# mpsops/mps-bitsandbytes

Measured on AMD Instinct MI355X. Metric: effective bf16 TFLOPS, NF4 dequant+matmul 4096x4096 @ M=4096 (dequantise-once + dense GEMM, two launches), higher is better.
Workload: dtype bf16

## Files before the change

mps_bitsandbytes_amd/csrc/common.h:

```cpp
#pragma once

#include <hip/hip_runtime.h>
#include <stdint.h>

#include "../../include/mbnb_hip.h"
#include "elem_types.h"

namespace mbnb {

template <int DT> struct ElemT;
template <> struct ElemT<MBNB_F16> { using type = f16_t; };
template <> struct ElemT<MBNB_BF16> { using type = bf16_t; };
template <> struct ElemT<MBNB_F32> { using type = float; };

template <typename T> __device__ __forceinline__ float to_f32(T v) { return (float)v; }
template <typename T> __device__ __forceinline__ T from_f32(float v) { return (T)v; }
template <> __device__ __forceinline__ f16_t from_f32<f16_t>(float v) {
    asm("" : "+v"(v));
    return (f16_t)v;
}

typedef uint32_t u32x4 __attribute__((ext_vector_type(4)));
typedef uint32_t u32x2 __attribute__((ext_vector_type(2)));
typedef float f32x4 __attribute__((ext_vector_type(4)));
// ... 15 lines not shown
template <> __device__ __forceinline__ uint32_t pack2<bf16_t>(float lo, float hi) {
    bf16x2 v = {(bf16_t)lo, (bf16_t)hi};
    return __builtin_bit_cast(uint32_t, v);
}

template <typename T> __device__ __forceinline__ float unpack_lo(uint32_t w);
template <typename T> __device__ __forceinline__ float unpack_hi(uint32_t w);
template <> __device__ __forceinline__ float unpack_lo<f16_t>(uint32_t w) {
    return (float)__builtin_bit_cast(f16x2, w)[0];
}
template <> __device__ __forceinline__ float unpack_hi<f16_t>(uint32_t w) {
    return (float)__builtin_bit_cast(f16x2, w)[1];
}
template <> __device__ __forceinline__ float unpack_lo<bf16_t>(uint32_t w) {
    return __builtin_bit_cast(float, w << 16);
}
template <> __device__ __forceinline__ float unpack_hi<bf16_t>(uint32_t w) {
    return __builtin_bit_cast(float, w & 0xFFFF0000u);
}

__device__ __forceinline__ float nf4_code(int i) {
    constexpr float t[16] = {-1.0f, -0.6961928009986877f, -0.5250730514526367f, -0.39491748809814453f,
                             -0.28444138169288635f, -0.18477343022823334f, -0.09105003625154495f, 0.0f,
                             0.07958029955625534f, 0.16093020141124725f, 0.24611230194568634f,
                             0.33791524171829224f, 0.44070982933044434f, 0.5626170039176941f,
                             0.7229568362236023f, 1.0f};
    return t[i];
}
__device__ __forceinline__ float fp4_code(int i) {
    constexpr float t[16] = {0.0f, 0.0625f, 0.125f, 0.25f, 0.375f, 0.5f, 0.75f, 1.0f,
                             -0.0f, -0.0625f, -0.125f, -0.25f, -0.375f, -0.5f, -0.75f, -1.0f};
    return t[i];
}
template <int QT> __device__ __forceinline__ float code_value(int i) {
    return QT == MBNB_NF4 ? nf4_code(i) : fp4_code(i);
}

template <int QT> __device__ __forceinline__ void fill_code_lut(float *lut, int tid) {
    if (tid < 16) {
        float v = 0.0f;
#pragma unroll
        for (int i = 0; i < 16; i++)
            if (tid == i) v = code_value<QT>(i);
        lut[tid] = v;
    }
}

constexpr int W8_INT8 = 0, W8_FP8 = 1;

__device__ __forceinline__ float fp8_e4m3_to_float(uint32_t b) {
    const uint32_t t = b << 24;
    const uint32_t u = (t & 0x80000000u) | ((t >> 4) & 0x07F00000u);
    float f = __builtin_bit_cast(float, u) * 0x1p120f;
    if ((t & 0x7F000000u) == 0x7F000000u) f = __builtin_bit_cast(float, 0x7FC00000u);
    return f;
}

__device__ __forceinline__ int fp8_exponent(float a) {
    const uint32_t u = __builtin_bit_cast(uint32_t, a);
    const uint32_t ef = (u >> 23) & 0xFFu;
    if (ef == 0) return -127;
    int e = (int)ef - 127;
    const int k = e + 1;
    const uint32_t n = k >= 9 ? 5u : k >= 5 ? 2u : k >= 3 ? 1u : k >= -1 ? 0u : k >= -3 ? 1u : k >= -7 ? 2u : k >= -15 ? 5u : 11u;
    if ((0x7FFFFFu - (u & 0x7FFFFFu)) < n) e += 1;
    return e;
}

__device__ __forceinline__ uint32_t float_to_fp8_e4m3(float v) {
    if (v != v) return 0x7Fu;
    const uint32_t sign = v < 0.0f ? 0x80u : 0u;
    const uint32_t ab = __builtin_bit_cast(uint32_t, fminf(fabsf(v), 448.0f));
    if (ab == 0u) return sign;
    const int k = (int)(ab >> 23) - 126;
    const uint32_t m = ab & 0x7FFFFFu;
    const int t = 2 * k - 1, at = t < 0 ? -t : t;
    const uint32_t n = at >= 9 ? 2u : (at >= 5 ? 1u : 0u);
    const bool bump = (0x7FFFFFu - m) < n;
    const int biased = k + 6 + (bump ? 1 : 0);
    if (biased >= 15) return sign | 0x77u;
    if (biased <= 0) return sign;
    uint32_t mb = (m + 0x80000u) >> 20;
    mb = bump ? 0u : (mb > 7u ? 7u : mb);
    return sign | ((uint32_t)biased << 3) | mb;
}

struct OutlierEpilogue {
    const void *x;
    int64_t ldx;
    const int64_t *oidx;
    int64_t n_out;
    const void *ow;
    const void *bias;
};

template <int WF> __device__ __forceinline__ float w8_row_scale(float s) { return WF == W8_INT8 ? s / 127.0f : s; }
template <int WF> __device__ __forceinline__ float w8_decode(uint32_t byte) {
    if constexpr (WF == W8_INT8) return (float)(int)(int8_t)byte;
    else return fp8_e4m3_to_float(byte);
}
template <int WF> __device__ __forceinline__ float w8_decode_sel(uint32_t word, int sel) {
    if constexpr (WF == W8_INT8) {
        return (float)(int)(int8_t)(word >> (8 * sel));
    } else {
        switch (sel) {
            case 0: return __builtin_amdgcn_cvt_f32_fp8((int)word, 0);
            case 1: return __builtin_amdgcn_cvt_f32_fp8((int)word, 1);
            case 2: return __builtin_amdgcn_cvt_f32_fp8((int)word, 2);
            default: return __builtin_amdgcn_cvt_f32_fp8((int)word, 3);
        }
    }
}

struct AbsmaxView {
    const float *f32;
    const int8_t *i8;
    const float *am2;
    int bs2;
};

template <bool NESTED> __device__ __forceinline__ float load_absmax(const AbsmaxView &a, int64_t i) {
    if constexpr (NESTED) {
        float s = a.am2[i / a.bs2] / 127.0f;
        return (float)a.i8[i] * s;
    } else {
        return a.f32[i];
    }
}

__device__ __forceinline__ float rscale127(float absmax) {
    float r = 1.0f / absmax;
    return r * 127.0f;
}

__device__ __forceinline__ int8_t quant_i8(float x, float scale) {
    float q = rintf(x * scale);
    q = fminf(fmaxf(q, -127.0f), 127.0f);
    return (int8_t)(int)q;
}

__device__ __forceinline__ float wave_max(float v) {
#pragma unroll
    for (int off = 32; off > 0; off >>= 1) v = fmaxf(v, __shfl_xor(v, off, 64));
    return v;
}
__device__ __forceinline__ float wave_sum(float v) {
#pragma unroll
    for (int off = 32; off > 0; off >>= 1) v += __shfl_xor(v, off, 64);
    return v;
}

constexpr int MBNB_NOT_APPLICABLE = -1000;

__device__ __forceinline__ void store_f32x4_wt(float *dst, f32x4 v) { asm volatile("global_store_dwordx4 %0, %1, off sc1" ::"v"(dst), "v"(v) : "memory"); }
__device__ __forceinline__ void store_out16_nt(u32x4 *dst, u32x4 v) { __builtin_nontemporal_store(v, dst); }
__device__ __forceinline__ void store_out16(u32x4 *dst, u32x4 v) {
    asm volatile("global_store_dwordx4 %0, %1, off sc1" ::"v"(dst), "v"(v) : "memory");
}
void set_error(const char *fmt, ...);
void set_kernel_name(const char *name);
void set_kernel_variant(const char *fmt, ...) __attribute__((format(printf, 1, 2)));
int check_launch(const char *what);
int ensure_dyn_lds(const void *func, int bytes, const char *what);

}
```

mps_bitsandbytes_amd/csrc/gemm_dense.h:

```cpp
#pragma once
#include "gemm256.h"
#include <type_traits>
#include <utility>

namespace mbnb {

template <int... I, class F> __device__ __forceinline__ void gd_static_for_impl(std::integer_sequence<int, I...>, F &&f) {
    (f(std::integral_constant<int, I>{}), ...);
}
template <int N, class F> __device__ __forceinline__ void gd_static_for(F &&f) {
    gd_static_for_impl(std::make_integer_sequence<int, N>{}, static_cast<F &&>(f));
}

constexpr int GD_LDS = 4 * P_IMG;

template <int FM, int FN = 8> struct GdPlan {
    static_assert(FN == 8 || (FM == 8 && FN >= 5 && FN <= 7), "narrow tiles exist for the 256-row tile only");
    static constexpr int NS = 2 * FN * FM, NR = FN + FM, NP = FN + FM;
    static constexpr int RS1 = (FM == 8 && FN >= 7) ? 2 : 1;
    static constexpr int B1 = FM != 8 ? 16 : (FN == 8 ? 36 : FN == 7 ? 32 : FN == 6 ? 16 : 13), D0 = B1;
    static constexpr int DS = FM == 8 ? 4 : 2;
    static constexpr int B2 = FM != 8 ? 42 : (FN == 8 ? 100 : FN == 7 ? 94 : FN == 6 ? 78 : 66), R0 = B2;
    static_assert(R0 >= FN * FM, "the next tile's slice 0 replaces this tile's only after its MFMAs");
    static_assert((NR - 1) * RS1 < B1, "slice 1 is in registers before barrier 1");
// ... 45 lines not shown

    typedef int i32x4_t __attribute__((ext_vector_type(4)));
    i32x4_t rs_a, rs_b;
    {
        const uint64_t pa = reinterpret_cast<uint64_t>(X + m0 * K + k_begin), pb = reinterpret_cast<uint64_t>(Wd + n0 * ldw + k_begin);
        const int64_t rows_a = M - m0 < TM ? M - m0 : TM, rows_b = N - n0 < TN ? N - n0 : TN;
        rs_a = i32x4_t{(int)(uint32_t)pa, (int)(uint32_t)(pa >> 32), (int)(rows_a * K * 2), 0x00020000};
        rs_b = i32x4_t{(int)(uint32_t)pb, (int)(uint32_t)(pb >> 32), (int)(rows_b * ldw * 2), 0x00020000};
    }
    int voff_a[FM], voff_b[FN];
#pragma unroll
    for (int pl = 0; pl < FN; pl++) {
        const int row = 8 * (FN * wave + pl) + (lane >> 3);
        voff_b[pl] = (int)(row * ldw * 2) + 16 * ((lane & 7) ^ ((row >> 1) & 7));
    }
#pragma unroll
    for (int pl = 0; pl < FM; pl++) {
        const int row = 8 * (FM * wave + pl) + (lane >> 3);
        voff_a[pl] = (int)(row * K * 2) + 16 * ((lane & 7) ^ ((row >> 1) & 7));
    }
#pragma unroll
    for (int pl = 0; pl < FN; pl++) voff_b[pl] -= (pl & 3) * 1024;
#pragma unroll
    for (int pl = 0; pl < FM; pl++) voff_a[pl] -= (pl & 3) * 1024;
    const uint32_t smem_base = (uint32_t)(uintptr_t)(__attribute__((address_space(3))) void *)smem;
    struct DmaCtx { i32x4_t ra, rb; uint32_t lwa, lwb; };
    auto dma_ctx = [&]() {
        DmaCtx c;
#pragma unroll
        for (int e = 0; e < 4; e++) {
            c.ra[e] = __builtin_amdgcn_readfirstlane(rs_a[e]);
            c.rb[e] = __builtin_amdgcn_readfirstlane(rs_b[e]);
        }
        c.lwa = (uint32_t)__builtin_amdgcn_readfirstlane((int)(smem_base + (uint32_t)(P_A + wave * FM * 1024)));
        c.lwb = (uint32_t)__builtin_amdgcn_readfirstlane((int)(smem_base + (uint32_t)(P_B + wave * FN * 1024)));
        return c;
    };
    auto issue_piece = [&](auto qq, int stage, int kb, const DmaCtx &c) {
        constexpr int q = decltype(qq)::value, pl = q < FM ? q : q - FM;
        const uint32_t dst = (q < FM ? c.lwa : c.lwb) + (uint32_t)(stage * P_IMG + pl * 1024);
        const int vo = (q < FM) ? voff_a[pl] : voff_b[pl];
        const i32x4_t rs = (q < FM) ? c.ra : c.rb;
        if constexpr ((pl & 3) != 0) {
            asm volatile("buffer_load_dwordx4 %0, %1, %2 offen offset:%3 lds" ::"v"(vo), "s"(rs), "s"(kb), "n"((pl & 3) * 1024) : "memory", "m0");
        } else {
            asm volatile("s_mov_b32 m0, %0\n\ts_nop 0\n\tbuffer_load_dwordx4 %1, %2, %3 offen lds" ::"s"(dst), "v"(vo), "s"(rs), "s"(kb) : "memory", "m0");
        }
    };

    const int r16 = lane & 15, fq = lane >> 4;
    int fw[2], fx[2];
#pragma unroll
    for (int ks = 0; ks < 2; ks++) {
        const int f = r16 * ROW_BYTES + (((4 * ks + fq) ^ (r16 >> 1)) << 4);
        fw[ks] = P_B + wn * 16 * FN * ROW_BYTES + f;
        fx[ks] = P_A + wm * 16 * FM * ROW_BYTES + f;
    }
    Frag wf[2][FN], xf[2][FM];
    auto read_one = [&](int stage, auto kk, auto nn) {
        constexpr int ks = decltype(kk)::value, n = decltype(nn)::value;
        if constexpr (n == 0) wf[ks][0] = *reinterpret_cast<const Frag *>(smem + fw[ks] + stage * P_IMG);
        else if constexpr (n <= FM) xf[ks][n - 1] = *reinterpret_cast<const Frag *>(smem + fx[ks] + stage * P_IMG + (n - 1) * 16 * ROW_BYTES);
        else wf[ks][n - FM] = *reinterpret_cast<const Frag *>(smem + fw[ks] + stage * P_IMG + (n - FM) * 16 * ROW_BYTES);
    };
    f32x4 acc[FN][FM];

    auto kbytes = [&](int t) { return t << 7; };

    {
        const DmaCtx c0 = dma_ctx();
        gd_static_for<Plan::NP>([&](auto q) { issue_piece(q, 0, 0, c0); });
        if (nk > 1) {
            gd_static_for<Plan::NP>([&](auto q) { issue_piece(q, 1, kbytes(1), c0); });
            asm volatile("s_waitcnt vmcnt(%0)" ::"n"(Plan::NP) : "memory");
        } else {
            asm volatile("s_waitcnt vmcnt(0)" ::: "memory");
        }
    }
    __builtin_amdgcn_s_barrier();
    asm volatile("" ::: "memory");
    gd_static_for<Plan::NR>([&](auto n) { read_one(0, std::integral_constant<int, 0>{}, n); });

    auto mfma_acc = [&](f32x4 &c, const Frag &a, const Frag &b) {
        if constexpr (I8) asm volatile("v_mfma_i32_16x16x64_i8 %0, %1, %2, %0" : "+a"(c) : "v"(a), "v"(b));
        else if constexpr (std::is_same_v<T, bf16_t>) asm volatile("v_mfma_f32_16x16x32_bf16 %0, %1, %2, %0" : "+a"(c) : "v"(a), "v"(b));
        else asm volatile("v_mfma_f32_16x16x32_f16 %0, %1, %2, %0" : "+a"(c) : "v"(a), "v"(b));
    };
    auto mfma_zero = [&](f32x4 &c, const Frag &a, const Frag &b) {
        if constexpr (I8) asm volatile("v_mfma_i32_16x16x64_i8 %0, %1, %2, 0" : "=a"(c) : "v"(a), "v"(b));
        else if constexpr (std::is_same_v<T, bf16_t>) asm volatile("v_mfma_f32_16x16x32_bf16 %0, %1, %2, 0" : "=a"(c) : "v"(a), "v"(b));
        else asm volatile("v_mfma_f32_16x16x32_f16 %0, %1, %2, 0" : "=a"(c) : "v"(a), "v"(b));
    };

    auto kstep = [&](auto cc, auto first, auto mode_, auto wo_, int j, const DmaCtx &dc) {
        constexpr int WO = decltype(wo_)::value, MODE = decltype(mode_)::value;
        constexpr bool FIRST = decltype(first)::value;
        const int C = cc, Nn = C ^ 1;
        int kb2 = 0;
        if constexpr (MODE == 0) kb2 = __builtin_amdgcn_readfirstlane(kbytes(j + 2));
        gd_static_for<Plan::NS>([&](auto tt) {
            constexpr int t = decltype(tt)::value, ks = t / (FN * FM), f = (t % (FN * FM)) / FM, g = t % FM;
            if constexpr (t == Plan::B1 && MODE != 2) {
                asm volatile("s_waitcnt lgkmcnt(0)" ::: "memory");
                __builtin_amdgcn_s_barrier();
                asm volatile("" ::: "memory");
            }
            if constexpr (t == Plan::B2 && MODE != 2) {
                asm volatile("s_waitcnt vmcnt(%0)" ::"n"(MODE == 0 ? Plan::NP : 0) : "memory");
                __builtin_amdgcn_s_barrier();
                asm volatile("" ::: "memory");
            }
            if constexpr (FIRST && ks == 0) mfma_zero(acc[f][g], wf[ks][f], xf[ks][g]);
            else mfma_acc(acc[f][g], wf[ks][f], xf[ks][g]);
            if constexpr ((t % Plan::RS1) == 0 && t / Plan::RS1 < Plan::NR)
                read_one(C, std::integral_constant<int, 1>{}, std::integral_constant<int, (t / Plan::RS1) % Plan::NR>{});
            if constexpr (MODE != 2 && t >= Plan::R0 && t < Plan::R0 + Plan::NR)
                read_one(Nn, std::integral_constant<int, 0>{}, std::integral_constant<int, (t - Plan::R0) % Plan::NR>{});
            if constexpr (MODE == 0 && t >= Plan::D0 && t < Plan::D0 + Plan::NP * Plan::DS && ((t - Plan::D0) % Plan::DS) == WO)
                issue_piece(std::integral_constant<int, ((t - Plan::D0) / Plan::DS) % Plan::NP>{}, C, kb2, dc);
            __builtin_amdgcn_sched_barrier(0);
        });
    };
    using Mode0 = std::integral_constant<int, 0>;
    using Mode1 = std::integral_constant<int, 1>;
    using Mode2 = std::integral_constant<int, 2>;
    auto main_loop = [&](auto wo) {
        if (nk < 3) return;
        const DmaCtx dc = dma_ctx();
        kstep(std::integral_constant<int, 0>{}, std::true_type{}, Mode0{}, wo, 0, dc);
        int j = 1;
        for (; j + 3 < nk; j += 2) {
            kstep(std::integral_constant<int, 1>{}, std::false_type{}, Mode0{}, wo, j, dc);
            kstep(std::integral_constant<int, 0>{}, std::false_type{}, Mode0{}, wo, j + 1, dc);
        }
        if (j + 2 < nk) kstep(std::integral_constant<int, 1>{}, std::false_type{}, Mode0{}, wo, j, dc);
    };
    if constexpr (Plan::DS == 4) {
        if (wave == 0) main_loop(std::integral_constant<int, 0>{});
        else if (wave == 1) main_loop(std::integral_constant<int, 1>{});
        else if (wave == 2) main_loop(std::integral_constant<int, 2>{});
        else main_loop(std::integral_constant<int, 3>{});
    } else {
        if ((wave & 1) == 0) main_loop(std::integral_constant<int, 0>{});
        else main_loop(std::integral_constant<int, 1>{});
    }

    constexpr bool TAIL = !SPLITK && !I8 && OUTL == 0 && FN == 8;
    bool tail_ok = false;
    if constexpr (TAIL)
        tail_ok = nk >= 2 && out_dtype == (std::is_same_v<T, f16_t> ? MBNB_F16 : MBNB_BF16) && (N % 8 == 0) &&
                  ((reinterpret_cast<uintptr_t>(out_v) & 15) == 0) && N < ((int64_t)1 << 23);
    u32x2 bias_t[TAIL ? FN : 1];
    if constexpr (TAIL) {
        if (tail_ok && bias != nullptr) {
            const uint16_t *bp = reinterpret_cast<const uint16_t *>(bias);
#pragma unroll
            for (int f = 0; f < FN; f++) {
                const int64_t n = n0 + wn * 16 * FN + 16 * f + 4 * fq;
                if (n + 4 <= N && (reinterpret_cast<uintptr_t>(bp + n) & 7) == 0) bias_t[f] = *reinterpret_cast<const u32x2 *>(bp + n);
                else {
                    uint32_t t[4];
#pragma unroll
                    for (int e = 0; e < 4; e++) t[e] = bp[n + e < N ? n + e : N - 1];
                    bias_t[f] = u32x2{t[0] | (t[1] << 16), t[2] | (t[3] << 16)};
                }
            }
        }
    }
    {
        const DmaCtx none{};
        if (nk == 2) kstep(std::integral_constant<int, 0>{}, std::true_type{}, Mode1{}, std::integral_constant<int, 0>{}, 0, none);
        else if (nk > 2) kstep(nk & 1, std::false_type{}, Mode1{}, std::integral_constant<int, 0>{}, nk - 2, none);
        if (nk == 1) kstep(std::integral_constant<int, 0>{}, std::true_type{}, Mode2{}, std::integral_constant<int, 0>{}, 0, none);
        else if (!tail_ok) kstep((nk - 1) & 1, std::false_type{}, Mode2{}, std::integral_constant<int, 0>{}, nk - 1, none);
    }
    if constexpr (TAIL) {
        auto tail_step = [&](auto wb_t, const int C) {
            constexpr bool WB = decltype(wb_t)::value;
            constexpr int ROWB = 264, GS = 2 * FN;
            int tid2 = threadIdx.x;
            asm volatile("" : "+v"(tid2));
            const int lane_e = tid2 & 63, er16 = lane_e & 15, efq = lane_e >> 4;
            char *stg = smem + (wn ? P_B : P_A) + (C ^ 1) * P_IMG + wm * (2 * 16 * ROWB);
            char *st_w = stg + er16 * ROWB + 8 * efq;
            const char *st_r = stg + efq * ROWB + er16 * 16;
            const int64_t m_w = m0 + wm * 16 * FM;
            int64_t rows = M - m_w;
            rows = rows < 0 ? 0 : (rows > 16 * FM ? 16 * FM : rows);
            const uint64_t po = reinterpret_cast<uint64_t>(static_cast<uint16_t *>(out_v) + m_w * N);
            i32x4_t rs_o;
            rs_o[0] = __builtin_amdgcn_readfirstlane((int)(uint32_t)po);
            rs_o[1] = __builtin_amdgcn_readfirstlane((int)(uint32_t)(po >> 32));
            rs_o[2] = __builtin_amdgcn_readfirstlane((int)(rows * N * 2));
            rs_o[3] = 0x00020000;
            const int rowstep = __builtin_amdgcn_readfirstlane((int)(N * 2));
            const int64_t n = n0 + wn * 16 * FN + er16 * 8;
            const int voff0 = n < N ? (int)((efq * N + n) * 2) : (int)0x80000000;
            u32x4 piece[4];
            auto filler = [&](auto gg, auto ss) {
                constexpr int g = decltype(gg)::value, s = decltype(ss)::value, buf = (g & 1) * 16 * ROWB;
                if constexpr (s < FN) {
                    float bv[4] = {0.0f, 0.0f, 0.0f, 0.0f};
                    if constexpr (WB) {
#pragma unroll
                        for (int e = 0; e < 4; e++) bv[e] = unpack_lo<T>(bias_t[s][e >> 1] >> (16 * (e & 1)));
                    }
                    float v[4];
#pragma unroll
                    for (int e = 0; e < 4; e++) {
                        float sv;
                        asm volatile("v_accvgpr_read_b32 %0, %1" : "=v"(sv) : "a"(acc[s][g][e]));
                        v[e] = sv + bv[e];
                    }
                    const u32x2 pk = u32x2{pack2<T>(v[0], v[1]), pack2<T>(v[2], v[3])};
                    *reinterpret_cast<u32x2 *>(st_w + buf + 32 * s) = pk;
                } else if constexpr (s < FN + 4) {
                    constexpr int p = s - FN;
                    const char *srcp = st_r + buf + p * 4 * ROWB;
                    const u32x2 lo = *reinterpret_cast<const u32x2 *>(srcp), hi = *reinterpret_cast<const u32x2 *>(srcp + 8);
                    piece[p] = u32x4{lo[0], lo[1], hi[0], hi[1]};
                } else if constexpr (s < FN + 8) {
                    constexpr int p = s - FN - 4;
                    const int vo = voff0 + (16 * g + 4 * p) * rowstep;
                    const i32x4_t rs = rs_o;
                    const u32x4 pv = piece[p];
                    asm volatile("buffer_store_dwordx4 %0, %1, %2, 0 offen sc1\n\ts_nop 1" ::"v"(pv), "v"(vo), "s"(rs) : "memory");
                }
            };
            gd_static_for<Plan::NS>([&](auto tt) {
                constexpr int t = decltype(tt)::value, g = t / GS, ks = (t % GS) / FN, f = t % FN;
                if constexpr (std::is_same_v<T, bf16_t>) asm volatile("s_nop 1\n\tv_mfma_f32_16x16x32_bf16 %0, %1, %2, %0" : "+a"(acc[f][g]) : "v"(wf[ks][f]), "v"(xf[ks][g]));
                else asm volatile("s_nop 1\n\tv_mfma_f32_16x16x32_f16 %0, %1, %2, %0" : "+a"(acc[f][g]) : "v"(wf[ks][f]), "v"(xf[ks][g]));
                if constexpr (t < Plan::NR)
                    read_one(C, std::integral_constant<int, 1>{},
                             std::integral_constant<int, (t == 0 ? 1 : t == 1 ? 0 : t <= FN ? t - 1 + FM : t - FN + 1)>{});
                if constexpr (t >= GS) filler(std::integral_constant<int, t / GS - 1>{}, std::integral_constant<int, t % GS>{});
                __builtin_amdgcn_sched_barrier(0);
            });
            gd_static_for<GS>([&](auto ss) {
                filler(std::integral_constant<int, FM - 1>{}, ss);
                __builtin_amdgcn_sched_barrier(0);
            });
        };
        if (tail_ok) {
            if (bias != nullptr) tail_step(std::true_type{}, (nk - 1) & 1);
            else tail_step(std::false_type{}, (nk - 1) & 1);
            return;
        }
    }

    asm volatile("s_waitcnt lgkmcnt(0)" ::: "memory");
    __builtin_amdgcn_s_barrier();
    asm volatile("" ::: "memory");
    int tid2 = threadIdx.x;
    asm volatile("" : "+v"(tid2));
    const int lane_e = tid2 & 63, er16 = lane_e & 15, efq = lane_e >> 4;
    const int64_t n_base = n0 + wn * 16 * FN;
    if constexpr (SPLITK) {
        float *o = partial + (int64_t)slice * M * N;
#pragma unroll
        for (int f = 0; f < FN; f++)
#pragma unroll
            for (int g = 0; g < FM; g++) {
                const int64_t m = m0 + wm * 16 * FM + 16 * g + er16, nn = n_base + 16 * f + 4 * efq;
                float v[4];
#pragma unroll
                for (int e = 0; e < 4; e++) asm volatile("v_accvgpr_read_b32 %0, %1" : "=v"(v[e]) : "a"(acc[f][g][e]));
                if (m < M && nn < N) store4_partial(o + m * N + nn, v, nn, N);
                __builtin_amdgcn_sched_barrier(0);
            }
        return;
    }
    if (out_dtype == MBNB_F32) {
        float *o = static_cast<float *>(out_v);
#pragma unroll
        for (int f = 0; f < FN; f++)
#pragma unroll
            for (int g = 0; g < FM; g++) {
                const int64_t m = m0 + wm * 16 * FM + 16 * g + er16, nn = n_base + 16 * f + 4 * efq;
                float v[4];
#pragma unroll
                for (int e = 0; e < 4; e++) {
                    float sv;
                    asm volatile("v_accvgpr_read_b32 %0, %1" : "=v"(sv) : "a"(acc[f][g][e]));
                    if constexpr (I8) {
                        v[e] = (float)__builtin_bit_cast(int, sv) * (sA[m < M ? m : M - 1] / 127.0f) * (sB[nn + e < N ? nn + e : N - 1] / 127.0f);
                    } else {
                        if (bias != nullptr && nn + e < N) sv += to_f32(bias[nn + e]);
                        v[e] = to_f32(from_f32<T>(sv));
                    }
                }
                if (m < M && nn < N) store4(o + m * N + nn, v, nn, N);
                __builtin_amdgcn_sched_barrier(0);
            }
        return;
    }
    constexpr int ROWB = 264;
    char *wave_lds = smem + wave * 64 * ROWB;
    uint16_t *out = static_cast<uint16_t *>(out_v);
    const bool vec_ok = (N % 8 == 0) && ((reinterpret_cast<uintptr_t>(out_v) & 15) == 0);
    const bool same_out = !I8 && out_dtype == (std::is_same_v<T, f16_t> ? MBNB_F16 : MBNB_BF16);
    const bool with_outl = OUTL != 0 && ep.x != nullptr && ep.n_out > 0;
    const bool ow_vec = OUTL != 0 && (ep.n_out % 8 == 0) && ((reinterpret_cast<uintptr_t>(ep.ow) & 15) == 0);
    using OutlT = std::conditional_t<OUTL == 1, f16_t, bf16_t>;
    auto rne = [&](float x) { return to_f32(from_f32<OutlT>(x)); };
    u32x4 wfr_all[OUTL ? 8 * NCH : 1];
    u32x2 bias_all[(OUTL || !I8) ? FN : 1];
    u32x4 xfr_all[OUTL ? FM * NCH : 1];
    if constexpr (!I8) {
        if (bias != nullptr) {
            const uint16_t *bp = reinterpret_cast<const uint16_t *>(bias);
#pragma unroll
            for (int f = 0; f < FN; f++) {
                const int64_t n = n_base + 16 * f + 4 * efq;
                if (n + 4 <= N && (reinterpret_cast<uintptr_t>(bp + n) & 7) == 0) bias_all[f] = *reinterpret_cast<const u32x2 *>(bp + n);
                else {
                    uint32_t t[4];
#pragma unroll
                    for (int e = 0; e < 4; e++) t[e] = bp[n + e < N ? n + e : N - 1];
                    bias_all[f] = u32x2{t[0] | (t[1] << 16), t[2] | (t[3] << 16)};
                }
            }
        }
    }
    if constexpr (OUTL) {
#pragma unroll
        for (int f = 0; f < 8; f++) {
            bias_all[f] = u32x2{0u, 0u};
#pragma unroll
            for (int c = 0; c < NCH; c++) {
                wfr_all[8 * c + f] = u32x4{0u, 0u, 0u, 0u};
                if (with_outl) {
                    const uint16_t *ow = static_cast<const uint16_t *>(ep.ow);
                    int64_t n = n_base + 16 * f + er16;
                    n = n < N ? n : N - 1;
                    const int64_t j0 = 32 * c + 8 * efq;
                    if (ow_vec && j0 + 8 <= ep.n_out) wfr_all[8 * c + f] = *reinterpret_cast<const u32x4 *>(ow + n * ep.n_out + j0);
                    else if (j0 < ep.n_out) {
                        uint32_t t[8];
#pragma unroll
                        for (int e = 0; e < 8; e++) t[e] = (j0 + e < ep.n_out) ? (uint32_t)ow[n * ep.n_out + j0 + e] : 0u;
                        wfr_all[8 * c + f] = u32x4{t[0] | (t[1] << 16), t[2] | (t[3] << 16), t[4] | (t[5] << 16), t[6] | (t[7] << 16)};
                    }
                }
            }
            if (ep.bias != nullptr) {
                const uint16_t *bp = static_cast<const uint16_t *>(ep.bias);
                const int64_t n = n_base + 16 * f + 4 * efq;
                if (n + 4 <= N && (reinterpret_cast<uintptr_t>(bp + n) & 7) == 0) bias_all[f] = *reinterpret_cast<const u32x2 *>(bp + n);
                else {
                    uint32_t t[4];
#pragma unroll
                    for (int e = 0; e < 4; e++) t[e] = bp[n + e < N ? n + e : N - 1];
                    bias_all[f] = u32x2{t[0] | (t[1] << 16), t[2] | (t[3] << 16)};
                }
            }
        }
#pragma unroll
        for (int g = 0; g < FM; g++) {
#pragma unroll
            for (int c = 0; c < NCH; c++) {
                xfr_all[FM * c + g] = u32x4{0u, 0u, 0u, 0u};
                if (with_outl) {
                    const uint16_t *xx = static_cast<const uint16_t *>(ep.x);
                    int64_t m = m0 + wm * 16 * FM + 16 * g + er16;
                    m = m < M ? m : M - 1;
                    const int64_t j0 = 32 * c + 8 * efq;
                    if (j0 < ep.ldx) xfr_all[FM * c + g] = *reinterpret_cast<const u32x4 *>(xx + m * ep.ldx + j0);
                }
            }
        }
    }
    float bv_all[I8 ? FN : 1][4];
    if constexpr (I8) {
        const bool sb_vec = (reinterpret_cast<uintptr_t>(sB) & 15) == 0;
#pragma unroll
        for (int f = 0; f < FN; f++) {
            const int64_t n = n_base + 16 * f + 4 * efq;
            f32x4 t;
            if (sb_vec && n + 4 <= N) t = *reinterpret_cast<const f32x4 *>(sB + n);
            else {
#pragma unroll
                for (int e = 0; e < 4; e++) t[e] = sB[n + e < N ? n + e : N - 1];
            }
#pragma unroll
            for (int e = 0; e < 4; e++) bv_all[f][e] = t[e] / 127.0f;
        }
    }
    auto epilogue16 = [&](auto wo_t, auto wb_t) {
    constexpr bool WO = decltype(wo_t)::value, WB = decltype(wb_t)::value;
    constexpr int GP = 1;
    gd_static_for<FM / GP>([&](auto hh) {
        constexpr int H = decltype(hh)::value;
        const int64_t m_base = m0 + wm * 16 * FM + 16 * GP * H;
        float sa[GP] = {};
        if constexpr (I8) {
#pragma unroll
            for (int g = 0; g < GP; g++) {
                const int64_t m = m_base + 16 * g + er16;
// ... 146 lines not shown
```

mps_bitsandbytes_amd/csrc/quant_kernels.hip:

```cpp
#include "common.h"
#include "dispatch.h"

namespace mbnb {

template <typename T>
__device__ __forceinline__ void load8(const T *A, int64_t rows, int64_t cols, int64_t r, int64_t k0,
                                      bool vec_ok, float (&x)[8]) {
    if (vec_ok && k0 + 8 <= cols) {
        if constexpr (sizeof(T) == 2) {
            u32x4 v = *reinterpret_cast<const u32x4 *>(A + r * cols + k0);
#pragma unroll
            for (int j = 0; j < 4; j++) {
                x[2 * j] = unpack_lo<T>(v[j]);
                x[2 * j + 1] = unpack_hi<T>(v[j]);
            }
        } else {
            f32x4 v0 = *reinterpret_cast<const f32x4 *>(A + r * cols + k0);
            f32x4 v1 = *reinterpret_cast<const f32x4 *>(A + r * cols + k0 + 4);
#pragma unroll
            for (int j = 0; j < 4; j++) {
                x[j] = v0[j];
                x[4 + j] = v1[j];
            }
        }
// ... 775 lines not shown
static int launch_quantize_4bit(const void *A, int64_t rows, int64_t cols, int64_t cols_padded, int blocksize,
                                int qt, const float *absmax_in, uint8_t *packed, float *absmax_out,
                                hipStream_t st) {
    const T *a = static_cast<const T *>(A);
    if (blocksize < 8) {
        const int64_t nbytes = rows * cols_padded / 2;
        const unsigned grid = (unsigned)((nbytes + 255) / 256);
        if (qt == MBNB_NF4)
            hipLaunchKernelGGL((k_quantize_4bit_tiny<T, MBNB_NF4>), dim3(grid), dim3(256), 0, st, a, rows, cols,
                               cols_padded, blocksize, absmax_in, packed, absmax_out);
        else
            hipLaunchKernelGGL((k_quantize_4bit_tiny<T, MBNB_FP4>), dim3(grid), dim3(256), 0, st, a, rows, cols,
                               cols_padded, blocksize, absmax_in, packed, absmax_out);
        set_kernel_name("q4_tiny");
        return check_launch("quantize_4bit(tiny)");
    }
    const bool vec_ok = aligned16(A) && (cols % 8 == 0);
    const int span = blocksize > 512 ? blocksize : 512;
    const int64_t spans_per_row = (cols_padded + span - 1) / span;
    const int64_t waves = rows * spans_per_row;
    const bool row_grid = spans_per_row >= 4 && (spans_per_row + 3) / 4 <= 65535 && rows <= 0x7FFFFFFF;
    const bool two = row_grid && blocksize <= 512 && spans_per_row >= 8;
    const int64_t per_wg = two ? 8 : 4;
    const dim3 grid = row_grid ? dim3((unsigned)rows, (unsigned)((spans_per_row + per_wg - 1) / per_wg)) : dim3((unsigned)((waves + 3) / 4));
#define MBNB_Q4(QT, SPW)                                                                                           \
    hipLaunchKernelGGL((k_quantize_4bit<T, QT, SPW>), grid, dim3(256), 0, st, a, rows, cols, cols_padded, blocksize, \
                       absmax_in, packed, absmax_out, vec_ok, row_grid)
    if (qt == MBNB_NF4) {
        if (two) MBNB_Q4(MBNB_NF4, 2);
        else MBNB_Q4(MBNB_NF4, 1);
    } else {
        if (two) MBNB_Q4(MBNB_FP4, 2);
        else MBNB_Q4(MBNB_FP4, 1);
    }
#undef MBNB_Q4
    if (blocksize > 512) {
        if (row_grid) set_kernel_name(vec_ok ? "q4_big_rows" : "q4_big_rows_s");
        else set_kernel_name(vec_ok ? "q4_big" : "q4_big_s");
    } else if (two) set_kernel_name(vec_ok ? "q4_rows2" : "q4_rows2_s");
    else if (row_grid) set_kernel_name(vec_ok ? "q4_rows" : "q4_rows_s");
    else set_kernel_name(vec_ok ? "q4_wave" : "q4_wave_s");
    return check_launch("quantize_4bit");
}

template <typename T>
static int launch_quantize_4bit_dq(const void *A, int64_t rows, int64_t cols, int64_t cols_padded, int blocksize, int qt,
                                   uint8_t *packed, int8_t *am_codes, float *absmax2, hipStream_t st) {
    const T *a = static_cast<const T *>(A);
    const bool vec_ok = aligned16(A) && (cols % 8 == 0);
    const int64_t total = rows * (cols_padded / blocksize);
    const unsigned grid = (unsigned)((total + 255) / 256);
    if (qt == MBNB_NF4)
        hipLaunchKernelGGL((k_quantize_4bit_dq<T, MBNB_NF4>), dim3(grid), dim3(256), 0, st, a, rows, cols, cols_padded, blocksize,
                           packed, am_codes, absmax2, vec_ok);
    else
        hipLaunchKernelGGL((k_quantize_4bit_dq<T, MBNB_FP4>), dim3(grid), dim3(256), 0, st, a, rows, cols, cols_padded, blocksize,
                           packed, am_codes, absmax2, vec_ok);
    set_kernel_name(vec_ok ? "q4_dq" : "q4_dq_s");
    return check_launch("quantize_4bit(dq)");
}

int quantize_4bit_dq_dispatch(const void *A, int dtype, int64_t rows, int64_t cols, int64_t cols_padded, int blocksize,
                              int qt, uint8_t *packed, int8_t *am_codes, float *absmax2, hipStream_t st) {
    switch (dtype) {
        case MBNB_F16: return launch_quantize_4bit_dq<f16_t>(A, rows, cols, cols_padded, blocksize, qt, packed, am_codes, absmax2, st);
        case MBNB_BF16: return launch_quantize_4bit_dq<bf16_t>(A, rows, cols, cols_padded, blocksize, qt, packed, am_codes, absmax2, st);
        default: return launch_quantize_4bit_dq<float>(A, rows, cols, cols_padded, blocksize, qt, packed, am_codes, absmax2, st);
    }
}

int quantize_4bit_dispatch(const void *A, int dtype, int64_t rows, int64_t cols, int64_t cols_padded,
                           int blocksize, int qt, const float *absmax_in, uint8_t *packed, float *absmax_out,
                           hipStream_t st) {
    switch (dtype) {
        case MBNB_F16: return launch_quantize_4bit<f16_t>(A, rows, cols, cols_padded, blocksize, qt, absmax_in, packed, absmax_out, st);
        case MBNB_BF16: return launch_quantize_4bit<bf16_t>(A, rows, cols, cols_padded, blocksize, qt, absmax_in, packed, absmax_out, st);
        default: return launch_quantize_4bit<float>(A, rows, cols, cols_padded, blocksize, qt, absmax_in, packed, absmax_out, st);
    }
}

template <typename T, bool FP8, int UN>
__global__ __launch_bounds__(256) void k_dequantize_rows8_wt(const uint8_t *__restrict__ q, const float *__restrict__ scales, int64_t rows, int64_t cols,
                                                            T *__restrict__ out) {
    const int64_t c0 = ((int64_t)blockIdx.x * 256 + threadIdx.x) * 8;
    if (c0 >= cols) return;
    u32x2 w[UN];
    float s[UN];
#pragma unroll
    for (int u = 0; u < UN; u++) {
        const int64_t r = (int64_t)blockIdx.y * UN + u;
        const bool ok = r < rows;
        w[u] = ok ? *reinterpret_cast<const u32x2 *>(q + r * cols + c0) : u32x2{0u, 0u};
        const float sc = ok ? scales[r] : 0.0f;
        s[u] = FP8 ? sc : sc / 127.0f;
    }
#pragma unroll
    for (int u = 0; u < UN; u++) {
        const int64_t r = (int64_t)blockIdx.y * UN + u;
        if (r >= rows) continue;
        u32x4 o;
#pragma unroll
        for (int e = 0; e < 4; e++) {
            const float v0 = (FP8 ? w8_decode_sel<W8_FP8>(w[u][e >> 1], (2 * e) & 3) : w8_decode_sel<W8_INT8>(w[u][e >> 1], (2 * e) & 3)) * s[u];
            const float v1 = (FP8 ? w8_decode_sel<W8_FP8>(w[u][e >> 1], (2 * e + 1) & 3) : w8_decode_sel<W8_INT8>(w[u][e >> 1], (2 * e + 1) & 3)) * s[u];
            o[e] = pack2<T>(v0, v1);
        }
        asm volatile("global_store_dwordx4 %0, %1, off sc1" ::"v"(out + r * cols + c0), "v"(o) : "memory");
    }
}
template <bool FP8>
static bool launch_rows8_wt(const uint8_t *q, const float *scales, int64_t rows, int64_t cols, int out_dtype, void *out, hipStream_t st, int policy) {
    if (policy == 0 || (out_dtype != MBNB_F16 && out_dtype != MBNB_BF16) || cols % 8 != 0 || rows <= 0 || rows >= 65536 * 4 ||
        ((reinterpret_cast<uintptr_t>(q) & 7) | (reinterpret_cast<uintptr_t>(out) & 15)) != 0)
        return false;
    const unsigned gx = (unsigned)((cols / 8 + 255) / 256);
    if (policy == 2) {
        const dim3 grid(gx, (unsigned)((rows + 3) / 4));
        if (grid.y > 65535u) return false;
        if (out_dtype == MBNB_F16) hipLaunchKernelGGL((k_dequantize_rows8_wt<f16_t, FP8, 4>), grid, dim3(256), 0, st, q, scales, rows, cols, static_cast<f16_t *>(out));
        else hipLaunchKernelGGL((k_dequantize_rows8_wt<bf16_t, FP8, 4>), grid, dim3(256), 0, st, q, scales, rows, cols, static_cast<bf16_t *>(out));
    } else {
        const dim3 grid(gx, (unsigned)rows);
        if (grid.y > 65535u) return false;
        if (out_dtype == MBNB_F16) hipLaunchKernelGGL((k_dequantize_rows8_wt<f16_t, FP8, 1>), grid, dim3(256), 0, st, q, scales, rows, cols, static_cast<f16_t *>(out));
        else hipLaunchKernelGGL((k_dequantize_rows8_wt<bf16_t, FP8, 1>), grid, dim3(256), 0, st, q, scales, rows, cols, static_cast<bf16_t *>(out));
    }
    return true;
}

template <typename T, int QT, bool NESTED, int UN>
__global__ __launch_bounds__(256) void k_dequantize_4bit_flat(const uint8_t *__restrict__ packed, AbsmaxView am, int64_t ndw, int bs_shift,
                                                             T *__restrict__ out, int write_through) {
    __shared__ float lut[16];
    const int64_t base = (int64_t)blockIdx.x * (256 * UN) + threadIdx.x;
    uint32_t w[UN];
    float a[UN];
#pragma unroll
    for (int u = 0; u < UN; u++) {
        const int64_t g = base + 256 * u;
        const bool ok = g < ndw;
        w[u] = ok ? reinterpret_cast<const uint32_t *>(packed)[g] : 0u;
        a[u] = ok ? load_absmax<NESTED>(am, (g * 8) >> bs_shift) : 0.0f;
    }
    fill_code_lut<QT>(lut, threadIdx.x);
    __syncthreads();
#pragma unroll
    for (int u = 0; u < UN; u++) {
        const int64_t g = base + 256 * u;
        if (g >= ndw) continue;
        u32x4 p;
#pragma unroll
        for (int j = 0; j < 4; j++) p[j] = pack2<T>(lut[(w[u] >> (8 * j)) & 15] * a[u], lut[(w[u] >> (8 * j + 4)) & 15] * a[u]);
        u32x4 *o = reinterpret_cast<u32x4 *>(out) + g;
        if (write_through) asm volatile("global_store_dwordx4 %0, %1, off sc1" ::"v"(o), "v"(p) : "memory");
        else *o = p;
    }
}

template <typename T, int QT>
static int launch_dequantize_4bit(const uint8_t *packed, const AbsmaxView &am, int64_t rows, int64_t cols,
                                  int64_t cols_padded, int blocksize, void *out, hipStream_t st, int store_policy) {
    if constexpr (sizeof(T) == 2) {
        const int64_t ndw = rows * cols / 8;
        if (cols == cols_padded && cols % 8 == 0 && blocksize >= 8 && cols % blocksize == 0 && aligned16(out) &&
            (reinterpret_cast<uintptr_t>(packed) & 3) == 0 && ndw >= 65536 && (ndw + 255) / 256 <= 0x7FFFFFFF) {
            const int sh = __builtin_ctz((unsigned)blocksize);
            if (store_policy == 2) {
                const dim3 grid((unsigned)((ndw + 1023) / 1024));
                if (am.i8) hipLaunchKernelGGL((k_dequantize_4bit_flat<T, QT, true, 4>), grid, dim3(256), 0, st, packed, am, ndw, sh, static_cast<T *>(out), 1);
                else hipLaunchKernelGGL((k_dequantize_4bit_flat<T, QT, false, 4>), grid, dim3(256), 0, st, packed, am, ndw, sh, static_cast<T *>(out), 1);
            } else {
                const dim3 grid((unsigned)((ndw + 255) / 256));
                if (am.i8) hipLaunchKernelGGL((k_dequantize_4bit_flat<T, QT, true, 1>), grid, dim3(256), 0, st, packed, am, ndw, sh, static_cast<T *>(out), store_policy);
                else hipLaunchKernelGGL((k_dequantize_4bit_flat<T, QT, false, 1>), grid, dim3(256), 0, st, packed, am, ndw, sh, static_cast<T *>(out), store_policy);
            }
            set_kernel_name("dq4_flat");
            return check_launch("dequantize_4bit");
        }
    }
    const int64_t gpr = (cols + 7) / 8;
    const int64_t groups = rows * gpr;
    const bool row_grid = gpr >= 256 && (gpr + 255) / 256 <= 65535 && rows <= 0x7FFFFFFF;
    const dim3 grid = row_grid ? dim3((unsigned)rows, (unsigned)((gpr + 255) / 256)) : dim3((unsigned)((groups + 255) / 256));
    const bool vec_ok = aligned16(out) && (cols % 8 == 0);
    if (am.i8)
        hipLaunchKernelGGL((k_dequantize_4bit<T, QT, true>), grid, dim3(256), 0, st, packed, am, rows, cols,
                           cols_padded, blocksize, static_cast<T *>(out), vec_ok, row_grid);
    else
        hipLaunchKernelGGL((k_dequantize_4bit<T, QT, false>), grid, dim3(256), 0, st, packed, am, rows, cols,
                           cols_padded, blocksize, static_cast<T *>(out), vec_ok, row_grid);
    if (row_grid) set_kernel_name(vec_ok ? "dq4_rows" : "dq4_rows_s");
    else set_kernel_name(vec_ok ? "dq4_plain" : "dq4_plain_s");
    return check_launch("dequantize_4bit");
}

int dequantize_4bit_dispatch(const uint8_t *packed, const AbsmaxView &am, int64_t rows, int64_t cols,
                             int64_t cols_padded, int blocksize, int qt, int out_dtype, void *out,
                             hipStream_t st, int store_policy) {
#define MBNB_DQ(T)                                                                                              \
    (qt == MBNB_NF4 ? launch_dequantize_4bit<T, MBNB_NF4>(packed, am, rows, cols, cols_padded, blocksize, out, st, store_policy) \
                    : launch_dequantize_4bit<T, MBNB_FP4>(packed, am, rows, cols, cols_padded, blocksize, out, st, store_policy))
    switch (out_dtype) {
        case MBNB_F16: return MBNB_DQ(f16_t);
        case MBNB_BF16: return MBNB_DQ(bf16_t);
        default: return MBNB_DQ(float);
    }
#undef MBNB_DQ
}

int quantize_blockwise_dispatch(const void *A, int dtype, int64_t numel, int blocksize, const float *absmax_in,
                                int8_t *out, float *absmax_out, hipStream_t st) {
    if (absmax_in == nullptr && numel > 0 && numel % blocksize == 0 && blocksize >= 64)
        return quantize_rowwise_dispatch(A, dtype, numel / blocksize, blocksize, out, absmax_out, st);
    const unsigned grid = (unsigned)((numel + blocksize - 1) / blocksize);
    switch (dtype) {
        case MBNB_F16: hipLaunchKernelGGL(k_quantize_blockwise<f16_t>, dim3(grid), dim3(256), 0, st, static_cast<const f16_t *>(A), numel, blocksize, absmax_in, out, absmax_out); break;
        case MBNB_BF16: hipLaunchKernelGGL(k_quantize_blockwise<bf16_t>, dim3(grid), dim3(256), 0, st, static_cast<const bf16_t *>(A), numel, blocksize, absmax_in, out, absmax_out); break;
        default: hipLaunchKernelGGL(k_quantize_blockwise<float>, dim3(grid), dim3(256), 0, st, static_cast<const float *>(A), numel, blocksize, absmax_in, out, absmax_out); break;
    }
    set_kernel_name("q8_block");
    return check_launch("quantize_blockwise");
}

int dequantize_blockwise_dispatch(const int8_t *q, int64_t numel, const float *absmax, int blocksize, int out_dtype,
                                  void *out, hipStream_t st) {
    if (numel > 0 && numel % blocksize == 0 && blocksize >= 1024 && blocksize % 16 == 0 && numel / blocksize < 65536)
        return dequantize_rowwise_dispatch(q, absmax, numel / blocksize, blocksize, out_dtype, out, st);
    const unsigned grid = (unsigned)((numel + 255) / 256);
    switch (out_dtype) {
        case MBNB_F16: hipLaunchKernelGGL(k_dequantize_blockwise<f16_t>, dim3(grid), dim3(256), 0, st, q, numel, absmax, blocksize, static_cast<f16_t *>(out)); break;
        case MBNB_BF16: hipLaunchKernelGGL(k_dequantize_blockwise<bf16_t>, dim3(grid), dim3(256), 0, st, q, numel, absmax, blocksize, static_cast<bf16_t *>(out)); break;
        default: hipLaunchKernelGGL(k_dequantize_blockwise<float>, dim3(grid), dim3(256), 0, st, q, numel, absmax, blocksize, static_cast<float *>(out)); break;
    }
    set_kernel_name("dq8_block");
    return check_launch("dequantize_blockwise");
}

int quantize_rowwise_dispatch(const void *A, int dtype, int64_t rows, int64_t cols, int8_t *out, float *scales,
                              hipStream_t st) {
    const bool vec_ok = aligned16(A) && aligned16(out) && (cols % 8 == 0);
    const unsigned grid = (unsigned)rows;
    if (vec_ok && cols <= 8192 && dtype != MBNB_F32) {
        if (dtype == MBNB_F16) hipLaunchKernelGGL(k_quantize_rowwise_regs<f16_t>, dim3(grid), dim3(256), 0, st, static_cast<const f16_t *>(A), cols, out, scales);
        else hipLaunchKernelGGL(k_quantize_rowwise_regs<bf16_t>, dim3(grid), dim3(256), 0, st, static_cast<const bf16_t *>(A), cols, out, scales);
        set_kernel_name("q8_row_regs");
        return check_launch("quantize_rowwise");
    }
    switch (dtype) {
        case MBNB_F16: hipLaunchKernelGGL(k_quantize_rowwise<f16_t>, dim3(grid), dim3(256), 0, st, static_cast<const f16_t *>(A), rows, cols, out, scales, vec_ok); break;
        case MBNB_BF16: hipLaunchKernelGGL(k_quantize_rowwise<bf16_t>, dim3(grid), dim3(256), 0, st, static_cast<const bf16_t *>(A), rows, cols, out, scales, vec_ok); break;
        default: hipLaunchKernelGGL(k_quantize_rowwise<float>, dim3(grid), dim3(256), 0, st, static_cast<const float *>(A), rows, cols, out, scales, vec_ok); break;
    }
    set_kernel_name(vec_ok ? "q8_row_loop" : "q8_row_scalar");
    return check_launch("quantize_rowwise");
}

int quantize_fp8_dispatch(const void *A, int dtype, int64_t rows, int64_t cols, uint8_t *out, float *scales, hipStream_t st) {
    const bool vec_ok = (cols % 8 == 0) && ((reinterpret_cast<uintptr_t>(A) & 15) == 0) && ((reinterpret_cast<uintptr_t>(out) & 7) == 0);
    const unsigned grid = (unsigned)rows;
    switch (dtype) {
        case MBNB_F16: hipLaunchKernelGGL(k_quantize_fp8<f16_t>, dim3(grid), dim3(256), 0, st, static_cast<const f16_t *>(A), rows, cols, out, scales, vec_ok); break;
        case MBNB_BF16: hipLaunchKernelGGL(k_quantize_fp8<bf16_t>, dim3(grid), dim3(256), 0, st, static_cast<const bf16_t *>(A), rows, cols, out, scales, vec_ok); break;
        default: hipLaunchKernelGGL(k_quantize_fp8<float>, dim3(grid), dim3(256), 0, st, static_cast<const float *>(A), rows, cols, out, scales, vec_ok); break;
    }
    set_kernel_name(vec_ok ? "qfp8_row_loop" : "qfp8_row_scalar");
    return check_launch("quantize_fp8_e4m3");
}

int dequantize_fp8_dispatch(const uint8_t *q, const float *scales, int64_t rows, int64_t cols, int out_dtype, void *out,
                            hipStream_t st, int store_policy) {
    if (launch_rows8_wt<true>(q, scales, rows, cols, out_dtype, out, st, store_policy)) return check_launch("dequantize_fp8_e4m3");
    if (cols % 16 == 0 && ((reinterpret_cast<uintptr_t>(q) | reinterpret_cast<uintptr_t>(out)) & 15) == 0 && rows * cols > 0 && rows < 65536) {
        const dim3 g16((unsigned)((cols / 16 + 255) / 256), (unsigned)rows);
        switch (out_dtype) {
            case MBNB_F16: hipLaunchKernelGGL((k_dequantize_rows16<f16_t, true>), dim3(g16), dim3(256), 0, st, q, scales, rows, cols, static_cast<f16_t *>(out)); break;
            case MBNB_BF16: hipLaunchKernelGGL((k_dequantize_rows16<bf16_t, true>), dim3(g16), dim3(256), 0, st, q, scales, rows, cols, static_cast<bf16_t *>(out)); break;
            default: hipLaunchKernelGGL((k_dequantize_rows16<float, true>), dim3(g16), dim3(256), 0, st, q, scales, rows, cols, static_cast<float *>(out)); break;
        }
        set_kernel_name("dqfp8_rows16");
        return check_launch("dequantize_fp8_e4m3");
    }
    const unsigned grid = (unsigned)((rows * cols + 255) / 256);
    switch (out_dtype) {
        case MBNB_F16: hipLaunchKernelGGL(k_dequantize_fp8<f16_t>, dim3(grid), dim3(256), 0, st, q, scales, rows, cols, static_cast<f16_t *>(out)); break;
        case MBNB_BF16: hipLaunchKernelGGL(k_dequantize_fp8<bf16_t>, dim3(grid), dim3(256), 0, st, q, scales, rows, cols, static_cast<bf16_t *>(out)); break;
        default: hipLaunchKernelGGL(k_dequantize_fp8<float>, dim3(grid), dim3(256), 0, st, q, scales, rows, cols, static_cast<float *>(out)); break;
    }
    set_kernel_name("dqfp8_scalar");
    return check_launch("dequantize_fp8_e4m3");
}

int dequantize_rowwise_dispatch(const int8_t *q, const float *scales, int64_t rows, int64_t cols, int out_dtype,
                                void *out, hipStream_t st, int store_policy) {
    if (launch_rows8_wt<false>(reinterpret_cast<const uint8_t *>(q), scales, rows, cols, out_dtype, out, st, store_policy)) return check_launch("dequantize_rowwise");
    if (cols % 16 == 0 && ((reinterpret_cast<uintptr_t>(q) | reinterpret_cast<uintptr_t>(out)) & 15) == 0 && rows * cols > 0 && rows < 65536) {
        const dim3 g16((unsigned)((cols / 16 + 255) / 256), (unsigned)rows);
        const uint8_t *qb = reinterpret_cast<const uint8_t *>(q);
        switch (out_dtype) {
            case MBNB_F16: hipLaunchKernelGGL((k_dequantize_rows16<f16_t, false>), dim3(g16), dim3(256), 0, st, qb, scales, rows, cols, static_cast<f16_t *>(out)); break;
            case MBNB_BF16: hipLaunchKernelGGL((k_dequantize_rows16<bf16_t, false>), dim3(g16), dim3(256), 0, st, qb, scales, rows, cols, static_cast<bf16_t *>(out)); break;
            default: hipLaunchKernelGGL((k_dequantize_rows16<float, false>), dim3(g16), dim3(256), 0, st, qb, scales, rows, cols, static_cast<float *>(out)); break;
        }
        set_kernel_name("dq8_rows16");
        return check_launch("dequantize_rowwise");
    }
    const unsigned grid = (unsigned)((rows * cols + 255) / 256);
    switch (out_dtype) {
// ... 55 lines not shown
```

Measured before the change: 1414.

## Restructure GEMM tail to fuse last two k-steps with interleaved epilogue stores

The tail path of the dense GEMM now covers the final two k-steps instead of only the last one. It interleaves the MFMAs of both steps with the shared-memory fragment reads and a finer-grained epilogue filler, which splits the accumulator read and the pack/store into separate slots. The goal is to hide epilogue store and LDS staging latency behind the remaining matrix math and to remove one pipeline drain. It also adds s_nop padding after the inline write-through global stores, possibly as a hazard fix, which may cost a few cycles per store. The new schedule needs more registers and changes the staging-buffer placement, so occupancy or correctness at the edges could suffer.

```diff
diff --git a/mps_bitsandbytes_amd/csrc/common.h b/mps_bitsandbytes_amd/csrc/common.h
--- a/mps_bitsandbytes_amd/csrc/common.h
+++ b/mps_bitsandbytes_amd/csrc/common.h
@@ -191,10 +191,10 @@
 
 constexpr int MBNB_NOT_APPLICABLE = -1000;
 
-__device__ __forceinline__ void store_f32x4_wt(float *dst, f32x4 v) { asm volatile("global_store_dwordx4 %0, %1, off sc1" ::"v"(dst), "v"(v) : "memory"); }
+__device__ __forceinline__ void store_f32x4_wt(float *dst, f32x4 v) { asm volatile("global_store_dwordx4 %0, %1, off sc1\n\ts_nop 1" ::"v"(dst), "v"(v) : "memory"); }
 __device__ __forceinline__ void store_out16_nt(u32x4 *dst, u32x4 v) { __builtin_nontemporal_store(v, dst); }
 __device__ __forceinline__ void store_out16(u32x4 *dst, u32x4 v) {
-    asm volatile("global_store_dwordx4 %0, %1, off sc1" ::"v"(dst), "v"(v) : "memory");
+    asm volatile("global_store_dwordx4 %0, %1, off sc1\n\ts_nop 1" ::"v"(dst), "v"(v) : "memory");
 }
 void set_error(const char *fmt, ...);
 void set_kernel_name(const char *name);
diff --git a/mps_bitsandbytes_amd/csrc/gemm_dense.h b/mps_bitsandbytes_amd/csrc/gemm_dense.h
--- a/mps_bitsandbytes_amd/csrc/gemm_dense.h
+++ b/mps_bitsandbytes_amd/csrc/gemm_dense.h
@@ -221,6 +221,8 @@
                   ((reinterpret_cast<uintptr_t>(out_v) & 15) == 0) && N < ((int64_t)1 << 23);
     u32x2 bias_t[TAIL ? FN : 1];
     if constexpr (TAIL) {
+#pragma unroll
+        for (int f = 0; f < FN; f++) bias_t[f] = u32x2{0u, 0u};
         if (tail_ok && bias != nullptr) {
             const uint16_t *bp = reinterpret_cast<const uint16_t *>(bias);
 #pragma unroll
@@ -236,21 +238,44 @@
             }
         }
     }
-    {
+    if (!tail_ok) {
         const DmaCtx none{};
         if (nk == 2) kstep(std::integral_constant<int, 0>{}, std::true_type{}, Mode1{}, std::integral_constant<int, 0>{}, 0, none);
         else if (nk > 2) kstep(nk & 1, std::false_type{}, Mode1{}, std::integral_constant<int, 0>{}, nk - 2, none);
         if (nk == 1) kstep(std::integral_constant<int, 0>{}, std::true_type{}, Mode2{}, std::integral_constant<int, 0>{}, 0, none);
-        else if (!tail_ok) kstep((nk - 1) & 1, std::false_type{}, Mode2{}, std::integral_constant<int, 0>{}, nk - 1, none);
+        else kstep((nk - 1) & 1, std::false_type{}, Mode2{}, std::integral_constant<int, 0>{}, nk - 1, none);
     }
     if constexpr (TAIL) {
-        auto tail_step = [&](auto wb_t, const int C) {
-            constexpr bool WB = decltype(wb_t)::value;
-            constexpr int ROWB = 264, GS = 2 * FN;
+        auto tail2 = [&](auto first_t, const int CA) {
+            constexpr bool FIRST = decltype(first_t)::value;
+            constexpr int ROWB = 264, GS = 4 * FN;
+            static_assert(2 * (FN + 8) <= GS, "a part's FN + 8 fillers, two slots each, fit into a group");
+            const int off_a = CA * P_IMG, off_b = (CA ^ 1) * P_IMG;
+            Frag wq[2][FN], xg[4];
+            auto read_w = [&](Frag &dst, int off, auto kk, auto ff) {
+                dst = *reinterpret_cast<const Frag *>(smem + fw[decltype(kk)::value] + off + decltype(ff)::value * 16 * ROW_BYTES);
+            };
+            auto read_x = [&](auto gg, auto ii) {
+                constexpr int g = decltype(gg)::value, i = decltype(ii)::value;
+                xg[i] = *reinterpret_cast<const Frag *>(smem + fx[i & 1] + (i < 2 ? off_a : off_b) + g * 16 * ROW_BYTES);
+            };
+            using I0 = std::integral_constant<int, 0>;
+            using I1 = std::integral_constant<int, 1>;
+            xg[0] = xf[0][0];
+            read_x(I0{}, I1{});
+            gd_static_for<FN>([&](auto f) { read_w(wf[1][decltype(f)::value], off_a, I1{}, f); });
+            float bias_f[FN][4];
+#pragma unroll
+            for (int f = 0; f < FN; f++)
+#pragma unroll
+                for (int e = 0; e < 4; e++) bias_f[f][e] = unpack_lo<T>(bias_t[f][e >> 1] >> (16 * (e & 1)));
+            asm volatile("s_waitcnt vmcnt(0)" ::: "memory");
+            __builtin_amdgcn_s_barrier();
+            asm volatile("" ::: "memory");
             int tid2 = threadIdx.x;
             asm volatile("" : "+v"(tid2));
             const int lane_e = tid2 & 63, er16 = lane_e & 15, efq = lane_e >> 4;
-            char *stg = smem + (wn ? P_B : P_A) + (C ^ 1) * P_IMG + wm * (2 * 16 * ROWB);
+            char *stg = smem + P_B + wn * P_IMG + wm * (2 * 16 * ROWB);
             char *st_w = stg + er16 * ROWB + 8 * efq;
             const char *st_r = stg + efq * ROWB + er16 * 16;
             const int64_t m_w = m0 + wm * 16 * FM;
@@ -266,23 +291,20 @@
             const int64_t n = n0 + wn * 16 * FN + er16 * 8;
             const int voff0 = n < N ? (int)((efq * N + n) * 2) : (int)0x80000000;
             u32x4 piece[4];
-            auto filler = [&](auto gg, auto ss) {
-                constexpr int g = decltype(gg)::value, s = decltype(ss)::value, buf = (g & 1) * 16 * ROWB;
-                if constexpr (s < FN) {
-                    float bv[4] = {0.0f, 0.0f, 0.0f, 0.0f};
-                    if constexpr (WB) {
-#pragma unroll
-                        for (int e = 0; e < 4; e++) bv[e] = unpack_lo<T>(bias_t[s][e >> 1] >> (16 * (e & 1)));
-                    }
-                    float v[4];
+            float v[4];
+            auto filler = [&](auto gg, auto ss, auto hh) {
+                constexpr int g = decltype(gg)::value, s = decltype(ss)::value, h = decltype(hh)::value, buf = (g & 1) * 16 * ROWB;
+                if constexpr (s < FN && h == 0) {
 #pragma unroll
                     for (int e = 0; e < 4; e++) {
                         float sv;
                         asm volatile("v_accvgpr_read_b32 %0, %1" : "=v"(sv) : "a"(acc[s][g][e]));
-                        v[e] = sv + bv[e];
+                        v[e] = sv + bias_f[s][e];
                     }
+                } else if constexpr (s < FN) {
                     const u32x2 pk = u32x2{pack2<T>(v[0], v[1]), pack2<T>(v[2], v[3])};
                     *reinterpret_cast<u32x2 *>(st_w + buf + 32 * s) = pk;
+                } else if constexpr (h != 0) {
                 } else if constexpr (s < FN + 4) {
                     constexpr int p = s - FN;
                     const char *srcp = st_r + buf + p * 4 * ROWB;
@@ -296,24 +318,38 @@
                     asm volatile("buffer_store_dwordx4 %0, %1, %2, 0 offen sc1\n\ts_nop 1" ::"v"(pv), "v"(vo), "s"(rs) : "memory");
                 }
             };
-            gd_static_for<Plan::NS>([&](auto tt) {
-                constexpr int t = decltype(tt)::value, g = t / GS, ks = (t % GS) / FN, f = t % FN;
-                if constexpr (std::is_same_v<T, bf16_t>) asm volatile("s_nop 1\n\tv_mfma_f32_16x16x32_bf16 %0, %1, %2, %0" : "+a"(acc[f][g]) : "v"(wf[ks][f]), "v"(xf[ks][g]));
-                else asm volatile("s_nop 1\n\tv_mfma_f32_16x16x32_f16 %0, %1, %2, %0" : "+a"(acc[f][g]) : "v"(wf[ks][f]), "v"(xf[ks][g]));
-                if constexpr (t < Plan::NR)
-                    read_one(C, std::integral_constant<int, 1>{},
-                             std::integral_constant<int, (t == 0 ? 1 : t == 1 ? 0 : t <= FN ? t - 1 + FM : t - FN + 1)>{});
-                if constexpr (t >= GS) filler(std::integral_constant<int, t / GS - 1>{}, std::integral_constant<int, t % GS>{});
+            gd_static_for<FM * GS>([&](auto tt) {
+                constexpr int t = decltype(tt)::value, g = t / GS, r = t % GS, tile = r / (2 * FN), ks = (r / FN) % 2, f = r % FN;
+                if constexpr (t == GS) {
+                    asm volatile("s_waitcnt lgkmcnt(0)" ::: "memory");
+                    __builtin_amdgcn_s_barrier();
+                    asm volatile("" ::: "memory");
+                }
+                if constexpr (FIRST && r < FN) mfma_zero(acc[f][g], wf[0][f], xg[0]);
+                else if constexpr (tile == 0) mfma_acc(acc[f][g], wf[ks][f], xg[ks]);
+                else mfma_acc(acc[f][g], wq[ks][f], xg[2 + ks]);
+                if constexpr (g == 0 && r <= 2 * FN + 1) {
+                    constexpr int q = r % (FN + 1);
+                    using KS = std::integral_constant<int, r / (FN + 1)>;
+                    if constexpr (q == 0) read_x(I0{}, std::integral_constant<int, 2 + KS::value>{});
+                    else read_w(wq[KS::value][q - 1], off_b, KS{}, std::integral_constant<int, q - 1>{});
+                }
+                if constexpr (g + 1 < FM && r >= FN + 3 && (r - 3) % FN == 0)
+                    read_x(std::integral_constant<int, (g + 1) % FM>{}, std::integral_constant<int, ((r - 3) / FN - 1) % 4>{});
+                if constexpr (g >= 1 && r == 3) read_x(std::integral_constant<int, g>{}, std::integral_constant<int, 3>{});
+                if constexpr (g >= 1 && r / 2 < FN + 8)
+                    filler(std::integral_constant<int, (g + FM - 1) % FM>{}, std::integral_constant<int, (r / 2) % (FN + 8)>{}, std::integral_constant<int, r & 1>{});
                 __builtin_amdgcn_sched_barrier(0);
             });
-            gd_static_for<GS>([&](auto ss) {
-                filler(std::integral_constant<int, FM - 1>{}, ss);
+            gd_static_for<FN + 8>([&](auto ss) {
+                filler(std::integral_constant<int, FM - 1>{}, ss, I0{});
+                filler(std::integral_constant<int, FM - 1>{}, ss, I1{});
                 __builtin_amdgcn_sched_barrier(0);
             });
         };
         if (tail_ok) {
-            if (bias != nullptr) tail_step(std::true_type{}, (nk - 1) & 1);
-            else tail_step(std::false_type{}, (nk - 1) & 1);
+            if (nk == 2) tail2(std::true_type{}, 0);
+            else tail2(std::false_type{}, nk & 1);
             return;
         }
     }
diff --git a/mps_bitsandbytes_amd/csrc/quant_kernels.hip b/mps_bitsandbytes_amd/csrc/quant_kernels.hip
--- a/mps_bitsandbytes_amd/csrc/quant_kernels.hip
+++ b/mps_bitsandbytes_amd/csrc/quant_kernels.hip
@@ -951,7 +951,7 @@
 #pragma unroll
         for (int j = 0; j < 4; j++) p[j] = pack2<T>(lut[(w[u] >> (8 * j)) & 15] * a[u], lut[(w[u] >> (8 * j + 4)) & 15] * a[u]);
         u32x4 *o = reinterpret_cast<u32x4 *>(out) + g;
-        if (write_through) asm volatile("global_store_dwordx4 %0, %1, off sc1" ::"v"(o), "v"(p) : "memory");
+        if (write_through) asm volatile("global_store_dwordx4 %0, %1, off sc1\n\ts_nop 1" ::"v"(o), "v"(p) : "memory");
         else *o = p;
     }
 }
```

New measurement: 1424 (median of 3 runs). Within noise of the previous version (+0.7%).
